# zd87pl/ai-crypto-trader

Hardware: AMD Instinct MI355X
Metric: backtested_1m_candles_per_sec_ga_pop_eval (higher is better)
Workload: dtype fp32; 1 GPU; model=ga_backtest_evolution, global_batch=1024, seq_len=1000000, parallelism=dp1, symbols=64, pop_per_gpu=1024, fitness_segments=64

## Files before the change

ai_crypto_trader_amd/ops/hip/backtest.hip:

```cpp

#include "bt_position.hpp"

namespace {

struct BtState {
    VoteState v;
    BtPosition pos;

    __device__ void load(const float* __restrict__ pr, float initial_equity)
    {
        v.load(pr);
        pos.load(pr, initial_equity);
        asm volatile("" : "+v"(v.will_os), "+v"(v.will_ob));
    }

    __device__ void step(int t, float4 c, float2 ms, float4 sv)
    {
#pragma clang fp contract(off)
        const int net = v.count<false>(
            t, c.x, v.recur<true>(t, c.x, c.w), ms, sv);
        pos.step<false>(t, net, v.entry_v, v.exit_v, c.x, c.y, c.z);
    }

    __device__ void warm(int t, float4 c)
    {
        v.recur<true>(t, c.x, c.w);
    }
};

#define BT_BBSUB 32
static_assert(BT_TILE % BT_BBSUB == 0, "sub-tiles must tile the tile");
static_assert(BT_WARMUP % BT_BBSUB == 0 && BT_WARMUP <= BT_TILE,
              "the warm-up is whole sub-tiles of the first tile");
static_assert(BT_BLOCK % BT_MAXWIN == 0 && BT_BBSUB <= BT_BLOCK &&
                  (BT_MAXWIN & (BT_MAXWIN - 1)) == 0,
              "a lane converts slots of one window only");
static_assert(BT_MAXWIN <= BT_WARMUP, "early-window entries are unused");

__device__ inline float4 bt_pack_sums(double a, double b)
{
    return make_float4(__int_as_float(__double2loint(a)),
                       __int_as_float(__double2hiint(a)),
                       __int_as_float(__double2loint(b)),
                       __int_as_float(__double2hiint(b)));
}

__device__ inline double bt_unpack_sum(float lo, float hi)
{
    return __hiloint2double(__float_as_int(hi), __float_as_int(lo));
}

template <bool HAS_RESNAP>
__global__ void __launch_bounds__(BT_BLOCK, 5) backtest_kernel(
    const float* __restrict__ candles,
    const float* __restrict__ pop,
    float* __restrict__ metrics,
    int nsym, int T, int P, int chunks_per_sym, float initial_equity)
{
#pragma clang fp contract(off)
    __shared__ float chist[BT_SPAN];
    __shared__ double csq[BT_SPAN];
    __shared__ float hl[BT_SPAN][2];
    __shared__ float4 rec[BT_TILE][2];
    __shared__ float4 bbtab[BT_BBSUB * BT_MAXWIN];
    __shared__ double sh_sum[BT_MAXWIN], sh_sum2[BT_MAXWIN];
    __shared__ double sh_invw[BT_MAXWIN];

    int sym, chunk;
    bt_block_map(blockIdx.x, nsym, chunks_per_sym, sym, chunk);
    const int tid = threadIdx.x;
    const int p = chunk * BT_BLOCK + tid;
    const bool act = p < P;

    BtState st;
    st.load(pop + (long)(act ? p : 0) * BT_NPARAM, initial_equity);
    const float4* my_bb = bbtab + (st.v.bb_w - 2);

    if (tid < BT_MAXWIN) {
        BollState b;
        b.init(tid + 2);
        sh_sum[tid] = b.sum;
        sh_sum2[tid] = b.sum2;
        sh_invw[tid] = b.inv_w;
    }
    if (tid < BT_BBSUB)
        bbtab[tid * BT_MAXWIN + BT_MAXWIN - 1] =
            make_float4(0.0f, 0.0f, 0.0f, 0.0f);

    const float4* sym_candles =
        reinterpret_cast<const float4*>(candles + (long)sym * T * 4);
    if (T > 0) st.v.ema_f = st.v.ema_s = sym_candles[0].x;

    for (int t0 = 0; t0 < T; t0 += BT_TILE) {
        int ltid = tid;
        asm volatile("" : "+v"(ltid));
        const int scan_w = ltid + 2;
        const bool is_scan = scan_w <= BT_MAXWIN;
        bt_stage_tile(sym_candles, t0, T, chist, hl, csq, ltid);
        const int tend = min(BT_TILE, T - t0);
        const bool resnap_tile = HAS_RESNAP && (t0 > 0) &&
                                 ((t0 & (BT_RESNAP - 1)) == 0);
        if (resnap_tile && is_scan) {
            BollState b;
            b.resnap(scan_w, &chist[BT_HALO]);
            sh_sum[ltid] = b.sum;
            sh_sum2[ltid] = b.sum2;
        }
        bt_shared_votes<true>(t0, tend, chist, hl, &rec[0][0], ltid);
        for (int s0 = 0; s0 < tend; s0 += BT_BBSUB) {
            const int send = min(s0 + BT_BBSUB, tend);
            const bool warm = t0 + s0 < BT_WARMUP;
            if (s0 > 0) __syncthreads();
            if (is_scan) {
                BollState b;
                b.sum = sh_sum[ltid];
                b.sum2 = sh_sum2[ltid];
#pragma unroll 4
                for (int tt = s0; tt < send; ++tt) {
                    const int i = tt + BT_HALO;
                    if (!(resnap_tile && tt == 0))
                        b.advance(chist[i], chist[i - scan_w], csq[i],
                                  csq[i - scan_w]);
                    bbtab[(tt - s0) * BT_MAXWIN + ltid] =
                        bt_pack_sums(b.sum, b.sum2);
                }
                sh_sum[ltid] = b.sum;
                sh_sum2[ltid] = b.sum2;
            }
            __syncthreads();
            if (warm) {
                for (int tt = s0; tt < send; ++tt)
                    st.warm(t0 + tt, rec[tt][0]);
                continue;
            }
            {
                BollState b;
                b.inv_w = sh_invw[ltid & (BT_MAXWIN - 1)];
                for (int e = ltid; e < (send - s0) * BT_MAXWIN;
                     e += BT_BLOCK) {
                    const float4 v = bbtab[e];
                    b.sum = bt_unpack_sum(v.x, v.y);
                    b.sum2 = bt_unpack_sum(v.z, v.w);
                    const float2 ms = b.stats<false>(0, 0);
                    bbtab[e].x = ms.x;
                    bbtab[e].y = ms.y;
                }
            }
            __syncthreads();
            for (int tt = s0; tt < send; ++tt) {
                const float4* e = &my_bb[(tt - s0) * BT_MAXWIN];
                st.step(t0 + tt, rec[tt][0], make_float2(e->x, e->y),
                        rec[tt][1]);
            }
        }
    }

    int otid = tid;
    asm volatile("" : "+v"(otid));
    const int po = chunk * BT_BLOCK + otid;
    if (po < P)
        st.pos.acc.finalize(metrics + ((long)po * nsym + sym) * BT_NMETRIC,
                            T);
}

}

extern "C" void launch_backtest(const float* candles, const float* pop,
                                float* metrics, int nsym, int T, int P,
                                float initial_equity, hipStream_t stream) {
    const int chunks = (P + BT_BLOCK - 1) / BT_BLOCK;
    auto k = T > BT_RESNAP ? backtest_kernel<true> : backtest_kernel<false>;
    hipLaunchKernelGGL(k, dim3(nsym * chunks), dim3(BT_BLOCK), 0, stream,
                       candles, pop, metrics, nsym, T, P, chunks,
                       initial_equity);
}
```

ai_crypto_trader_amd/ops/hip/bt_common.hpp:

```cpp
#pragma once

#include "common.hpp"

#define BT_BLOCK 256
#define BT_TILE 256
#define BT_NMETRIC 10
#define BT_FEE 0.001f
#define BT_EPS 1e-9f
#define BT_ANNUALIZE 0x1.6a7dccp+9f

__device__ __forceinline__ float bt_max(float a, float b)
{
    float r;
    asm("v_max_f32 %0, %1, %2" : "=v"(r) : "v"(a), "v"(b));
    return r;
}

__device__ __forceinline__ float bt_min(float a, float b)
{
    float r;
    asm("v_min_f32 %0, %1, %2" : "=v"(r) : "v"(a), "v"(b));
    return r;
}

__device__ __forceinline__ float bt_max_uniform(float uniform, float b)
{
    float r;
    asm("v_max_f32 %0, %1, %2" : "=v"(r) : "s"(uniform), "v"(b));
    return r;
}

__device__ __forceinline__ float bt_pos_part(float x)
{
    float r;
    asm("v_max_f32 %0, 0, %1" : "=v"(r) : "v"(x));
    return r;
}

__device__ __forceinline__ float bt_neg_part(float x)
{
    float r;
    asm("v_max_f32 %0, -%1, 0" : "=v"(r) : "v"(x));
    return r;
}

__device__ inline void bt_write_metrics(
    float* __restrict__ out, int T, float equity, float n_trades,
    float wins, float gross_p, float gross_l, float max_dd, float sum_ret,
    float sum_ret2)
{
#pragma clang fp contract(off)
    float n = (float)max(T, 1);
    float mean_r = sum_ret / n;
    float var_r = fmaxf(sum_ret2 / n - mean_r * mean_r, 0.0f);
    float sharpe = mean_r / fmaxf(sqrtf(var_r), BT_EPS) * BT_ANNUALIZE;
    if (!(n_trades > 0.0f)) sharpe = 0.0f;
    float win_rate = wins / fmaxf(n_trades, 1.0f);
    float fitness = (n_trades > 0.0f)
                        ? sharpe + win_rate - 2.0f * max_dd
                        : -1.0f;
    out[0] = equity; out[1] = n_trades; out[2] = wins;
    out[3] = gross_p; out[4] = gross_l; out[5] = max_dd;
    out[6] = sum_ret; out[7] = sum_ret2;
    out[8] = sharpe; out[9] = fitness;
}

struct BtAccum {
    float equity, max_eq, max_dd;
    float n_trades, wins, gross_p, gross_l;
    float sum_ret, sum_ret2;

    __device__ void init(float initial_equity)
    {
        equity = initial_equity; max_eq = initial_equity; max_dd = 0.f;
        n_trades = wins = gross_p = gross_l = 0.f;
        sum_ret = sum_ret2 = 0.f;
    }

    __device__ void trade(float pnl)
    {
        n_trades += 1.0f;
        wins += (pnl > 0.0f) ? 1.0f : 0.0f;
        gross_p += fmaxf(pnl, 0.0f);
        gross_l += fmaxf(-pnl, 0.0f);
    }

    __device__ void mark(float new_eq)
    {
#pragma clang fp contract(off)
        float r = new_eq / equity - 1.0f;
        sum_ret += r;
        sum_ret2 += r * r;
        equity = new_eq;
        max_eq = bt_max(max_eq, equity);
        max_dd = bt_max(max_dd, (max_eq - equity) / max_eq);
    }

    __device__ void finalize(float* __restrict__ out, int T) const
    {
        bt_write_metrics(out, T, equity, n_trades, wins, gross_p, gross_l,
                         max_dd, sum_ret, sum_ret2);
    }
};

__device__ inline void bt_block_map(int bid, int nsym, int chunks_per_sym,
                                    int& sym, int& chunk)
{
    int nblocks = nsym * chunks_per_sym;
    if ((nsym & 7) == 0 && (nblocks & 7) == 0) {
        int xcd = bid & 7, j = bid >> 3;
        sym = xcd + 8 * (j / chunks_per_sym);
        chunk = j % chunks_per_sym;
    } else {
        sym = bid / chunks_per_sym;
        chunk = bid % chunks_per_sym;
    }
}
```

ai_crypto_trader_amd/ops/hip/bt_vote.hpp:

```cpp
#pragma once

#include "bt_common.hpp"

#define BT_NPARAM 19
#define BT_MAXWIN 32
#define BT_HALO 64
#define BT_SPAN (BT_TILE + BT_HALO)
#define BT_WARMUP 128
#define BT_RESNAP 16384
#define BT_NSTATE 18

struct BollState {
    double sum, sum2, inv_w;

    __device__ void init(int w)
    {
        sum = sum2 = 0.0;
        inv_w = 1.0 / (double)w;
    }

    __device__ void resnap(int w, const float* __restrict__ hist)
    {
#pragma clang fp contract(off)
        double s = 0.0, s2 = 0.0;
        for (int j = BT_MAXWIN - 1; j >= 0; --j) {
            if (j < w) {
                double c = (double)hist[-j];
                s += c;
                s2 += c * c;
            }
        }
        sum = s;
        sum2 = s2;
    }

    __device__ void advance(float close, float oldc, double csq_new,
                            double csq_old)
    {
#pragma clang fp contract(off)
        double old = (double)oldc;
        double c64 = (double)close;
        sum += c64 - old;
        sum2 += csq_new - csq_old;
    }

    template <bool EARLY = true>
    __device__ float2 stats(int t, int w) const
    {
#pragma clang fp contract(off)
        double inv_cnt = inv_w;
        if (EARLY && t < BT_MAXWIN && t + 1 < w)
            inv_cnt = 1.0 / (t + 1.0);
        double mean64 = sum * inv_cnt;
        double var64 = fmax(sum2 * inv_cnt - mean64 * mean64, 0.0);
        return make_float2((float)mean64, sqrtf((float)var64));
    }
};

struct VoteState {
    float inv_rsi_p, rsi_os, rsi_ob;
    float a_f, a_s, a_sig;
    int bb_w;
    float bb_k, bb_bth, bb_sth;
    int entry_v, exit_v;
    float stoch_os, stoch_ob, will_os, will_ob;

    float ema_f, ema_s, sig;
    float avg_gain, avg_loss;
    BollState bb;

    __device__ void load(const float* __restrict__ pr)
    {
        inv_rsi_p = 1.0f / fmaxf(floorf(pr[0]), 1.0f);
        rsi_os = pr[1]; rsi_ob = pr[2];
        a_f = 2.0f / (pr[3] + 1.0f);
        a_s = 2.0f / (pr[4] + 1.0f);
        a_sig = 2.0f / (pr[5] + 1.0f);
        bb_w = min(max((int)pr[6], 2), BT_MAXWIN);
        bb_k = pr[7]; bb_bth = pr[8]; bb_sth = pr[9];
        entry_v = (int)pr[10]; exit_v = (int)pr[11];
        stoch_os = pr[17]; stoch_ob = pr[18];
        will_os = stoch_os - 100.0f;
        will_ob = stoch_ob - 100.0f;
        ema_f = ema_s = sig = 0.f;
        avg_gain = avg_loss = 0.f;
        bb.init(bb_w);
    }

    __device__ void resnap(const float* __restrict__ hist)
    {
        bb.resnap(bb_w, hist);
    }

    __device__ void warm_step(float close, float change)
    {
#pragma clang fp contract(off)
        ema_f += a_f * (close - ema_f);
        ema_s += a_s * (close - ema_s);
        float macd = ema_f - ema_s;
        sig += a_sig * (macd - sig);
        float gain = fmaxf(change, 0.0f);
        float loss = fmaxf(-change, 0.0f);
        avg_gain += (gain - avg_gain) * inv_rsi_p;
        avg_loss += (loss - avg_loss) * inv_rsi_p;
    }

    struct Osc { float macd_hist, rsi_num, rsi_den; };

    template <bool SEEDED = false>
    __device__ Osc recur(int t, float close, float change)
    {
#pragma clang fp contract(off)
        if (!SEEDED && t == 0) { ema_f = close; ema_s = close; }
        else {
            ema_f += a_f * (close - ema_f);
            ema_s += a_s * (close - ema_s);
        }
        float macd = ema_f - ema_s;
        sig += a_sig * (macd - sig);
        Osc o;
        o.macd_hist = macd - sig;

        float gain = SEEDED ? bt_pos_part(change) : fmaxf(change, 0.0f);
        float loss = SEEDED ? bt_neg_part(change) : fmaxf(-change, 0.0f);
        avg_gain += (gain - avg_gain) * inv_rsi_p;
        avg_loss += (loss - avg_loss) * inv_rsi_p;
        o.rsi_num = 100.0f * avg_gain;
        o.rsi_den = avg_gain + (SEEDED ? bt_max_uniform(BT_EPS, avg_loss)
                                       : fmaxf(avg_loss, BT_EPS));
        return o;
    }

    template <bool WARM_TEST = true>
    __device__ int count(int t, float close, Osc o, float2 ms,
                         float4 sv) const
    {
#pragma clang fp contract(off)
        float band = bb_k * ms.y;
        float bb_num = close - (ms.x - band);
        float bb_den = fmaxf(2.0f * band, BT_EPS);

        int net = 0;
        if (!WARM_TEST || t >= BT_WARMUP) {
            int buy = (o.rsi_num < rsi_os * o.rsi_den) +
                      (o.macd_hist > 0.0f) +
                      (bb_num < bb_bth * bb_den) +
                      (sv.x < stoch_os * sv.z) +
                      (sv.y < will_os * sv.z);
            int sell = (o.rsi_num > rsi_ob * o.rsi_den) +
                       (o.macd_hist < 0.0f) +
                       (bb_num > bb_sth * bb_den) +
                       (sv.x > stoch_ob * sv.z) +
                       (sv.y > will_ob * sv.z);
            net = buy - sell + __float_as_int(sv.w);
        }
        return net;
    }

    template <bool SKIP_BB>
    __device__ int step(int t, float close, float change, float oldc,
                        double csq_new, double csq_old, float4 sv)
    {
        const Osc o = recur(t, close, change);
        if (!SKIP_BB) bb.advance(close, oldc, csq_new, csq_old);
        return count(t, close, o, bb.stats(t, bb_w), sv);
    }
};

__device__ inline void bt_stage_tile(
    const float4* __restrict__ sym_candles, int t0, int T,
    float* __restrict__ chist, float (*__restrict__ hl)[2],
    double* __restrict__ csq, int tid = threadIdx.x)
{
#pragma clang fp contract(off)
    __syncthreads();
    for (int i = tid; i < BT_SPAN; i += BT_BLOCK) {
        const int t = t0 - BT_HALO + i;
        float4 c = make_float4(0.0f, 0.0f, 0.0f, 0.0f);
        if (t >= 0 && t < T) c = sym_candles[t];
        chist[i] = c.x;
        if (csq) csq[i] = (double)c.x * (double)c.x;
        hl[i][0] = c.y;
        hl[i][1] = c.z;
    }
    __syncthreads();
}

template <bool RECORD = false>
__device__ inline void bt_shared_votes(
    int t0, int tend, const float* __restrict__ chist,
    const float (*__restrict__ hl)[2], float4* __restrict__ sh_vote,
    int tid = threadIdx.x)
{
#pragma clang fp contract(off)
    if (tid >= tend) return;
    const int t = t0 + tid;
    const int base = tid + BT_HALO;
    const float cl = chist[base];
    const int L14 = min(t + 1, 14);
    float hmax = -1e30f, lmin = 1e30f;
    for (int j = 0; j < L14; ++j) {
        hmax = fmaxf(hmax, hl[base - j][0]);
        lmin = fminf(lmin, hl[base - j][1]);
    }
    const int L20 = min(t + 1, 20);
    double s20 = 0.0;
    for (int j = 0; j < L20; ++j) s20 += (double)chist[base - j];
    const float sma20 = (float)(s20 / (double)L20);
    const int L50 = min(t + 1, 50);
    double s50 = 0.0;
    for (int j = 0; j < L50; ++j) s50 += (double)chist[base - j];
    const float sma50 = (float)(s50 / (double)L50);
    const int trend = (cl > sma20 && sma20 > sma50) ? 1
                      : ((cl < sma20 && sma20 < sma50) ? -1 : 0);
    if (RECORD)
        sh_vote[2 * tid] = make_float4(
            cl, hl[base][0], hl[base][1],
            (t == 0) ? 0.0f : cl - chist[base - 1]);
    sh_vote[RECORD ? 2 * tid + 1 : tid] = make_float4(
        100.0f * (cl - lmin), -100.0f * (hmax - cl),
        fmaxf(hmax - lmin, BT_EPS), __int_as_float(trend));
}
```

Measured before the change: 440.6 billion candles/s.

## Precompute per-candle stochastic/Williams flip thresholds and skip redundant drawdown divides

Each candle's stochastic and Williams comparisons (sv.x < stoch_os*sv.z and the like) are turned into per-candle threshold values. A bisection over float bit patterns, shared across the block, finds the exact parameter value at which each comparison flips, so every population member then does one compare per signal with no multiply. The trend vote moves into the unused high/low staging buffer and is packed into the Bollinger table. The drawdown update also skips the division when the new drawdown cannot beat the current maximum, using a conservative multiply bound. Costs are the extra per-tile bisection work, added syncs, and a divergent branch in the equity update; the thresholds must stay bit-exact with the original comparisons.

```diff
diff --git a/ai_crypto_trader_amd/ops/hip/backtest.hip b/ai_crypto_trader_amd/ops/hip/backtest.hip
--- a/ai_crypto_trader_amd/ops/hip/backtest.hip
+++ b/ai_crypto_trader_amd/ops/hip/backtest.hip
@@ -14,11 +14,11 @@
         asm volatile("" : "+v"(v.will_os), "+v"(v.will_ob));
     }
 
-    __device__ void step(int t, float4 c, float2 ms, float4 sv)
+    __device__ void step(int t, float4 c, float2 ms, float4 sv, int trend)
     {
 #pragma clang fp contract(off)
-        const int net = v.count<false>(
-            t, c.x, v.recur<true>(t, c.x, c.w), ms, sv);
+        const int net = v.count<false, true>(
+            t, c.x, v.recur<true>(t, c.x, c.w), ms, sv, trend);
         pos.step<false>(t, net, v.entry_v, v.exit_v, c.x, c.y, c.z);
     }
 
@@ -62,6 +62,9 @@
     __shared__ double csq[BT_SPAN];
     __shared__ float hl[BT_SPAN][2];
     __shared__ float4 rec[BT_TILE][2];
+    int* trend = reinterpret_cast<int*>(&hl[0][0]);
+    static_assert(sizeof(int) * BT_TILE <= sizeof(float) * 2 * BT_SPAN,
+                  "the trend votes fit the dead high/low staging");
     __shared__ float4 bbtab[BT_BBSUB * BT_MAXWIN];
     __shared__ double sh_sum[BT_MAXWIN], sh_sum2[BT_MAXWIN];
     __shared__ double sh_invw[BT_MAXWIN];
@@ -106,7 +109,10 @@
             sh_sum[ltid] = b.sum;
             sh_sum2[ltid] = b.sum2;
         }
-        bt_shared_votes<true>(t0, tend, chist, hl, &rec[0][0], ltid);
+        const int my_trend =
+            bt_shared_votes<true>(t0, tend, chist, hl, &rec[0][0], ltid);
+        __syncthreads();
+        trend[ltid] = my_trend;
         for (int s0 = 0; s0 < tend; s0 += BT_BBSUB) {
             const int send = min(s0 + BT_BBSUB, tend);
             const bool warm = t0 + s0 < BT_WARMUP;
@@ -144,13 +150,15 @@
                     const float2 ms = b.stats<false>(0, 0);
                     bbtab[e].x = ms.x;
                     bbtab[e].y = ms.y;
+                    bbtab[e].z =
+                        __int_as_float(trend[s0 + e / BT_MAXWIN]);
                 }
             }
             __syncthreads();
             for (int tt = s0; tt < send; ++tt) {
                 const float4* e = &my_bb[(tt - s0) * BT_MAXWIN];
                 st.step(t0 + tt, rec[tt][0], make_float2(e->x, e->y),
-                        rec[tt][1]);
+                        rec[tt][1], __float_as_int(e->z));
             }
         }
     }
diff --git a/ai_crypto_trader_amd/ops/hip/bt_common.hpp b/ai_crypto_trader_amd/ops/hip/bt_common.hpp
--- a/ai_crypto_trader_amd/ops/hip/bt_common.hpp
+++ b/ai_crypto_trader_amd/ops/hip/bt_common.hpp
@@ -27,6 +27,13 @@
 {
     float r;
     asm("v_max_f32 %0, %1, %2" : "=v"(r) : "s"(uniform), "v"(b));
+    return r;
+}
+
+__device__ __forceinline__ float bt_mul_uniform(float uniform, float b)
+{
+    float r;
+    asm("v_mul_f32 %0, %1, %2" : "=v"(r) : "s"(uniform), "v"(b));
     return r;
 }
 
@@ -69,9 +76,12 @@
     float equity, max_eq, max_dd;
     float n_trades, wins, gross_p, gross_l;
     float sum_ret, sum_ret2;
+    float dd_c;
 
     __device__ void init(float initial_equity)
     {
+        dd_c = __int_as_float(__builtin_amdgcn_readfirstlane(__float_as_int(
+            (initial_equity >= 0x1p-100f) ? 0x1.fffffcp-1f : 0.0f)));
         equity = initial_equity; max_eq = initial_equity; max_dd = 0.f;
         n_trades = wins = gross_p = gross_l = 0.f;
         sum_ret = sum_ret2 = 0.f;
@@ -93,7 +103,9 @@
         sum_ret2 += r * r;
         equity = new_eq;
         max_eq = bt_max(max_eq, equity);
-        max_dd = bt_max(max_dd, (max_eq - equity) / max_eq);
+        const float x = max_eq - equity;
+        if (!(x <= max_eq * bt_mul_uniform(dd_c, max_dd)))
+            max_dd = bt_max(max_dd, x / max_eq);
     }
 
     __device__ void finalize(float* __restrict__ out, int T) const
diff --git a/ai_crypto_trader_amd/ops/hip/bt_vote.hpp b/ai_crypto_trader_amd/ops/hip/bt_vote.hpp
--- a/ai_crypto_trader_amd/ops/hip/bt_vote.hpp
+++ b/ai_crypto_trader_amd/ops/hip/bt_vote.hpp
@@ -131,9 +131,9 @@
         return o;
     }
 
-    template <bool WARM_TEST = true>
+    template <bool WARM_TEST = true, bool THETA = false>
     __device__ int count(int t, float close, Osc o, float2 ms,
-                         float4 sv) const
+                         float4 sv, int trend = 0) const
     {
 #pragma clang fp contract(off)
         float band = bb_k * ms.y;
@@ -144,15 +144,18 @@
         if (!WARM_TEST || t >= BT_WARMUP) {
             int buy = (o.rsi_num < rsi_os * o.rsi_den) +
                       (o.macd_hist > 0.0f) +
-                      (bb_num < bb_bth * bb_den) +
-                      (sv.x < stoch_os * sv.z) +
-                      (sv.y < will_os * sv.z);
+                      (bb_num < bb_bth * bb_den);
             int sell = (o.rsi_num > rsi_ob * o.rsi_den) +
                        (o.macd_hist < 0.0f) +
-                       (bb_num > bb_sth * bb_den) +
-                       (sv.x > stoch_ob * sv.z) +
-                       (sv.y > will_ob * sv.z);
-            net = buy - sell + __float_as_int(sv.w);
+                       (bb_num > bb_sth * bb_den);
+            if (THETA) {
+                buy += (stoch_os >= sv.x) + (will_os >= sv.z);
+                sell += (stoch_ob <= sv.y) + (will_ob <= sv.w);
+            } else {
+                buy += (sv.x < stoch_os * sv.z) + (sv.y < will_os * sv.z);
+                sell += (sv.x > stoch_ob * sv.z) + (sv.y > will_ob * sv.z);
+            }
+            net = buy - sell + (THETA ? trend : __float_as_int(sv.w));
         }
         return net;
     }
@@ -186,14 +189,63 @@
     __syncthreads();
 }
 
+#define BT_KEY_INF 0x7f800000
+__device__ __forceinline__ int bt_key(int k)
+{
+    return k >= 0 ? k : (int)(0x80000000u - (unsigned)k);
+}
+
+template <bool SELL>
+__device__ inline int bt_vote_flip(float num, float s, float est)
+{
+#pragma clang fp contract(off)
+    auto Q = [&](int k) {
+        const float f = __int_as_float(bt_key(k)) * s;
+        return SELL ? !(num > f) : (num < f);
+    };
+    const int KLOW = -BT_KEY_INF, KHIGH = BT_KEY_INF;
+    const int k0 = min(max(bt_key(__float_as_int(est)), KLOW + 1), KHIGH - 1);
+    int lo, hi;
+    unsigned step = 1;
+    if (Q(k0)) {
+        hi = k0; lo = KLOW;
+        while (step < (unsigned)hi - (unsigned)KLOW) {
+            const int c = hi - (int)step;
+            if (!Q(c)) { lo = c; break; }
+            hi = c; step <<= 1;
+        }
+    } else {
+        lo = k0; hi = KHIGH;
+        while (step < (unsigned)KHIGH - (unsigned)lo) {
+            const int c = lo + (int)step;
+            if (Q(c)) { hi = c; break; }
+            lo = c; step <<= 1;
+        }
+    }
+    while ((unsigned)hi - (unsigned)lo > 1u) {
+        const int mid = lo + (int)(((unsigned)hi - (unsigned)lo) >> 1);
+        if (Q(mid)) hi = mid; else lo = mid;
+    }
+    return hi;
+}
+
+__device__ inline float2 bt_vote_thresholds(float num, float s, float inv_s)
+{
+#pragma clang fp contract(off)
+    const float est = num * inv_s;
+    return make_float2(
+        __int_as_float(bt_key(bt_vote_flip<false>(num, s, est))),
+        __int_as_float(bt_key(bt_vote_flip<true>(num, s, est) - 1)));
+}
+
 template <bool RECORD = false>
-__device__ inline void bt_shared_votes(
+__device__ inline int bt_shared_votes(
     int t0, int tend, const float* __restrict__ chist,
     const float (*__restrict__ hl)[2], float4* __restrict__ sh_vote,
     int tid = threadIdx.x)
 {
 #pragma clang fp contract(off)
-    if (tid >= tend) return;
+    if (tid >= tend) return 0;
     const int t = t0 + tid;
     const int base = tid + BT_HALO;
     const float cl = chist[base];
@@ -213,11 +265,20 @@
     const float sma50 = (float)(s50 / (double)L50);
     const int trend = (cl > sma20 && sma20 > sma50) ? 1
                       : ((cl < sma20 && sma20 < sma50) ? -1 : 0);
-    if (RECORD)
+    const float st_num = 100.0f * (cl - lmin);
+    const float wl_num = -100.0f * (hmax - cl);
+    const float srange = fmaxf(hmax - lmin, BT_EPS);
+    if (RECORD) {
         sh_vote[2 * tid] = make_float4(
             cl, hl[base][0], hl[base][1],
             (t == 0) ? 0.0f : cl - chist[base - 1]);
-    sh_vote[RECORD ? 2 * tid + 1 : tid] = make_float4(
-        100.0f * (cl - lmin), -100.0f * (hmax - cl),
-        fmaxf(hmax - lmin, BT_EPS), __int_as_float(trend));
-}
+        const float inv_s = 1.0f / srange;
+        const float2 st = bt_vote_thresholds(st_num, srange, inv_s);
+        const float2 wl = bt_vote_thresholds(wl_num, srange, inv_s);
+        sh_vote[2 * tid + 1] = make_float4(st.x, st.y, wl.x, wl.y);
+    } else {
+        sh_vote[tid] = make_float4(st_num, wl_num, srange,
+                                   __int_as_float(trend));
+    }
+    return trend;
+}
```

After: 483.7 billion candles/s (median of 6 runs). +9.8%, better.
